# Kim-Dongjun/Soft-Truncation

Measured on AMD Instinct MI355X. Metric: training images/sec (DDPM++ CIFAR-10 32x32), higher is better.
Workload: dtype f32; 1 GPU; DDPM++ (VP) CIFAR-10 32x32, configs/vp/CIFAR10/ddpmpp_nll_st.py (BASELINE configs[1]); per_gpu_batch=128, global_batch=128, parallelism=dp1

## Files before the change

soft-truncation_amd/csrc/conv.hip:

```cpp
#include "igemm.h"
#include "stk_fp16.h"
#include "stk_fp16_train.h"

namespace {

using igemm::Cfg;
using igemm::MnMajor;
using igemm::keep_if;
using igemm::strip_row;

typedef __attribute__((address_space(1))) float gfloat;

struct ConvP {
  const float* x1; const float* x2; int C1, C2;
  const float* w; int w_layout;
  const float* bias; const float* temb; int temb_stride; const float* res; float inv_div; int use_div;
  float* y;
  const float* dy; float* dx1; float* dx2; float beta1, beta2, alpha;
  float* part; long part_stride;
  int N, H, W, Cin, Cout, OH, OW, KH, KW, stride, pad, sshift;
  int HW, OHW, taps;
  int ohw_shift, ow_shift;
};


template <int B, int KC, int LD>
struct RowChunk {
  static constexpr int PERQ = KC / 4, PASSES = B / 64, PER = PASSES * PERQ;
  static_assert(KC % 4 == 0 && B % 64 == 0 && PER <= 32, "bad RowChunk tile");
  const float* rowp[PASSES];
  unsigned rowbits;
  unsigned okm;
  int q, tid, Ktot;
  __device__ __forceinline__ void init(const float* base, long ld, int row0, int R, int Ktot_, int tid_) {
    tid = tid_; q = tid & 3; Ktot = Ktot_; rowbits = 0; okm = 0;
#pragma unroll
    for (int ps = 0; ps < PASSES; ++ps) {
      const int row = row0 + (tid >> 2) + 64 * ps;
      const bool ok = row < R;
      rowbits |= (ok ? 1u : 0u) << ps;
      rowp[ps] = base + (ok ? (long)row * ld : 0);
    }
  }
  __device__ __forceinline__ void load(int k0, float (&r)[PER]) {
    const int kb = k0 + q * PERQ;
    const bool kin = kb + PERQ <= Ktot;
    const int ko = kin ? kb : 0;
    okm = 0;
#pragma unroll
    for (int ps = 0; ps < PASSES; ++ps) {
      const float* s = rowp[ps] + ko;
#pragma unroll
      for (int j = 0; j < PERQ; ++j) r[ps * PERQ + j] = s[j];
      okm |= ((kin && ((rowbits >> ps) & 1u)) ? ((1u << PERQ) - 1u) : 0u) << (ps * PERQ);
    }
  }
  __device__ __forceinline__ void store(const float (&r)[PER], float* t) {
    if (okm == (PER == 32 ? 0xffffffffu : (1u << PER) - 1u)) {
#pragma unroll
      for (int ps = 0; ps < PASSES; ++ps)
#pragma unroll
        for (int j = 0; j < PERQ; ++j) t[(q * PERQ + j) * LD + (tid >> 2) + 64 * ps] = r[ps * PERQ + j];
    } else {
#pragma unroll
      for (int ps = 0; ps < PASSES; ++ps)
#pragma unroll
        for (int j = 0; j < PERQ; ++j)
          t[(q * PERQ + j) * LD + (tid >> 2) + 64 * ps] = keep_if(r[ps * PERQ + j], okm, ps * PERQ + j);
    }
  }
};

template <int B, int KC, int LD>
struct MnStrided {
  using Mp = MnMajor<B, KC>;
  static constexpr int PER = Mp::PER;
  const float* pm; long sk; int kg, tid, Ktot; bool ok;
  unsigned okm;
  __device__ __forceinline__ void init(const float* base, long smn, long sk_, int o0, int lim, int Ktot_, int tid_) {
    tid = tid_; sk = sk_; Ktot = Ktot_; okm = 0;
    const int mn = o0 + Mp::mn(tid);
    ok = mn < lim;
    pm = base + (ok ? (long)mn * smn : 0);
    kg = Mp::kgroup(tid) * PER;
  }
  __device__ __forceinline__ void load(int k0, float (&r)[PER]) {
    okm = 0;
#pragma unroll
    for (int i = 0; i < PER; ++i) {
      const int k = k0 + kg + i;
      const bool v = ok && k < Ktot;
      r[i] = pm[v ? (long)k * sk : 0];
      okm |= (v ? 1u : 0u) << i;
    }
  }
  __device__ __forceinline__ void store(const float (&r)[PER], float* t) {
#pragma unroll
    for (int i = 0; i < PER; ++i) t[(kg + i) * LD + Mp::mn(tid)] = keep_if(r[i], okm, i);
  }
};

template <class C>
struct AFwdK {
  RowChunk<C::BM, C::KC, C::LDA> rc;
  __device__ void init(const ConvP& p, int m0, int tid, int) { rc.init(p.w, (long)p.Cin * p.taps, m0, p.Cout, p.Cin * p.taps, tid); }
  __device__ void load(const ConvP&, int k0, float (&r)[C::NA]) { rc.load(k0, r); }
  __device__ void store(const float (&r)[C::NA], float* t) { rc.store(r, t); }
};
template <class C>
struct AFwdGen {
  MnStrided<C::BM, C::KC, C::LDA> ms;
  __device__ void init(const ConvP& p, int m0, int tid, int) { ms.init(p.w, (long)p.Cin * p.taps, 1, m0, p.Cout, p.Cin * p.taps, tid); }
  __device__ void load(const ConvP&, int k0, float (&r)[C::NA]) { ms.load(k0, r); }
  __device__ void store(const float (&r)[C::NA], float* t) { ms.store(r, t); }
};
template <class C>
struct AFwdNin {
  MnStrided<C::BM, C::KC, C::LDA> ms;
  __device__ void init(const ConvP& p, int m0, int tid, int) { ms.init(p.w, 1, p.Cout, m0, p.Cout, p.Cin, tid); }
  __device__ void load(const ConvP&, int k0, float (&r)[C::NA]) { ms.load(k0, r); }
  __device__ void store(const float (&r)[C::NA], float* t) { ms.store(r, t); }
};
template <class C>
struct ADgradNin {
  RowChunk<C::BM, C::KC, C::LDA> rc;
  __device__ void init(const ConvP& p, int m0, int tid, int) { rc.init(p.w, p.Cout, m0, p.Cin, p.Cout, tid); }
  __device__ void load(const ConvP&, int k0, float (&r)[C::NA]) { rc.load(k0, r); }
  __device__ void store(const float (&r)[C::NA], float* t) { rc.store(r, t); }
};
template <class C>
struct ADgradNinGen {
  MnStrided<C::BM, C::KC, C::LDA> ms;
  __device__ void init(const ConvP& p, int m0, int tid, int) { ms.init(p.w, p.Cout, 1, m0, p.Cin, p.Cout, tid); }
  __device__ void load(const ConvP&, int k0, float (&r)[C::NA]) { ms.load(k0, r); }
  __device__ void store(const float (&r)[C::NA], float* t) { ms.store(r, t); }
};
template <class C>
struct ADgrad1 {
  MnStrided<C::BM, C::KC, C::LDA> ms;
  __device__ void init(const ConvP& p, int m0, int tid, int) { ms.init(p.w, 1, p.Cin, m0, p.Cin, p.Cout, tid); }
  __device__ void load(const ConvP&, int k0, float (&r)[C::NA]) { ms.load(k0, r); }
  __device__ void store(const float (&r)[C::NA], float* t) { ms.store(r, t); }
};
template <class C>
struct ADgrad9 {
  static_assert(C::KC == 36, "3x3 chunks are 4 channels x 9 taps");
  static constexpr int PASSES = C::BM / 64;
  int m0, tid; unsigned okp;
  __device__ void init(const ConvP&, int m0_, int tid_, int) { m0 = m0_; tid = tid_; okp = 0; }
  __device__ void load(const ConvP& p, int k0, float (&r)[C::NA]) {
    const int co = k0 / 9 + (tid & 3);
    okp = 0;
#pragma unroll
    for (int ps = 0; ps < PASSES; ++ps) {
      const int m = m0 + (tid >> 2) + 64 * ps;
      const bool ok = m < p.Cin && co < p.Cout;
      const float* s = p.w + (ok ? ((long)co * p.Cin + m) * 9 : 0);
#pragma unroll
      for (int j = 0; j < 9; ++j) r[ps * 9 + j] = s[j];
      okp |= (ok ? 1u : 0u) << ps;
    }
  }
  __device__ void store(const float (&r)[C::NA], float* t) {
#pragma unroll
    for (int ps = 0; ps < PASSES; ++ps)
#pragma unroll
      for (int j = 0; j < 9; ++j)
        t[((tid & 3) * 9 + j) * C::LDA + (tid >> 2) + 64 * ps] = keep_if(r[ps * 9 + j], okp, ps);
  }
};

template <class C, int TAPS, bool DUAL>
// ... 169 lines not shown
    for (int i = 0; i < C::NB; ++i) {
      if (DUAL) {
        const bool f = (first >> i) & 1u;
        const uintptr_t tensor = f ? (uintptr_t)p.x1 : (uintptr_t)p.x2;
        r[i] = ((const gfloat*)tensor)[(f ? b1 : b2) + roff[i]];
      } else {
        r[i] = p.x1[b1 + roff[i]];
      }
    }
  }
  __device__ void store(const float (&r)[C::NB], float* t) {
#pragma unroll
    for (int i = 0; i < C::NB; ++i) t[(tid & 31) * C::LDB + (tid >> 5) + 8 * i] = keep_if(r[i], okm, i);
  }
};

struct EpFwd {
  int b; int col_off;
  static constexpr int TEMB_IMGS = 9;
  float rb; float rt[5]; int m0 = 0, b0 = 0, nimg = 0, tb = 0;
  const float* sb = nullptr; const float* stm = nullptr;
  __device__ void preload(const ConvP& p, int m0_, int n0, int tn, int M, int Nn, int tid) {
    m0 = m0_; sb = nullptr; stm = nullptr;
    b0 = n0 / p.OHW;
    nimg = min(n0 + tn - 1, Nn - 1) / p.OHW - b0 + 1;
    rb = (p.bias && tid < 128 && m0 + tid < M) ? p.bias[m0 + tid] : 0.f;
#pragma unroll
    for (int k = 0; k < 5; ++k) {
      const int idx = tid + 256 * k, img = idx >> 7, r = idx & 127;
      rt[k] = (p.temb && nimg <= TEMB_IMGS && img < nimg && m0 + r < M) ? p.temb[(long)(b0 + img) * p.temb_stride + m0 + r] : 0.f;
    }
  }
  __device__ void stage(unsigned char* lds, int tid) {
    __syncthreads();
    float* s = reinterpret_cast<float*>(lds);
    if (tid < 128) s[tid] = rb;
#pragma unroll
    for (int k = 0; k < 5; ++k) {
      const int idx = tid + 256 * k;
      if (idx < TEMB_IMGS * 128) s[128 + idx] = rt[k];
    }
    __syncthreads();
    sb = s; stm = s + 128;
  }
  __device__ void init(const ConvP&, int, int) {}
  __device__ void finish(const ConvP&, unsigned char*, int) {}
  __device__ void col(const ConvP& p, int n) {
    b = n / p.OHW;
    col_off = b * p.Cout * p.OHW + (n - b * p.OHW);
    tb = (b - b0) * 128;
  }
  __device__ void strip(const ConvP& p, int mbase, int M, bool nok, int, const floatx16& acc) {
    if (sb && (!p.temb || nimg <= TEMB_IMGS)) {
      const int ml = mbase - m0;
      float rv[16]; int idx[16];
#pragma unroll
      for (int e = 0; e < 16; ++e) {
        const int m = mbase + strip_row(e);
        const bool ok = nok && m < M;
        idx[e] = ok ? col_off + m * p.OHW : -1;
        rv[e] = (p.res && ok) ? p.res[idx[e]] : 0.f;
      }
#pragma unroll
      for (int g = 0; g < 4; ++g) {
        const float4 bb = *reinterpret_cast<const float4*>(sb + ml + 8 * g);
        const float4 tt = *reinterpret_cast<const float4*>(stm + tb + ml + 8 * g);
        const float bv[4] = {bb.x, bb.y, bb.z, bb.w}, tv[4] = {tt.x, tt.y, tt.z, tt.w};
#pragma unroll
        for (int u = 0; u < 4; ++u) {
          float v = acc[4 * g + u];
          if (p.bias) v += bv[u];
          if (p.temb) v += tv[u];
          if (p.res) v += rv[4 * g + u];
          if (p.use_div) v *= p.inv_div;
          if (idx[4 * g + u] >= 0) p.y[idx[4 * g + u]] = v;
        }
      }
      return;
    }
#pragma unroll
    for (int g = 0; g < 4; ++g) {
      float bv[4], tv[4], rv[4];
      int idx[4]; bool ok[4];
#pragma unroll
      for (int u = 0; u < 4; ++u) {
        const int m = mbase + strip_row(4 * g + u);
        ok[u] = nok && m < M;
        idx[u] = ok[u] ? col_off + m * p.OHW : 0;
        const int ms = ok[u] ? m : 0;
        bv[u] = p.bias ? p.bias[ms] : 0.f;
        tv[u] = p.temb ? p.temb[ok[u] ? (long)b * p.temb_stride + m : 0] : 0.f;
        rv[u] = p.res ? p.res[idx[u]] : 0.f;
      }
#pragma unroll
      for (int u = 0; u < 4; ++u) {
        float v = acc[4 * g + u];
        if (p.bias) v += bv[u];
        if (p.temb) v += tv[u];
        if (p.res) v += rv[u];
        if (p.use_div) v *= p.inv_div;
        if (ok[u]) p.y[idx[u]] = v;
      }
    }
  }
};
struct EpDgrad {
  int b, hw;
  __device__ void preload(const ConvP&, int, int, int, int, int, int) {}
  __device__ void stage(unsigned char*, int) {}
  __device__ void init(const ConvP&, int, int) {}
  __device__ void col(const ConvP& p, int n) { b = n / p.HW; hw = n - b * p.HW; }
  __device__ void strip(const ConvP& p, int mbase, int M, bool nok, int, const floatx16& acc) {
    const bool acc1 = p.beta1 != 0.f, acc2 = p.beta2 != 0.f;
#pragma unroll
    for (int e0 = 0; e0 < 16; e0 += 4) {
      float* d[4]; float old[4];
#pragma unroll
      for (int u = 0; u < 4; ++u) {
        const int m = mbase + strip_row(e0 + u);
        float* q = nullptr;
        if (nok && m < M) {
          if (m < p.C1) { if (p.dx1) q = p.dx1 + ((long)b * p.C1 + m) * p.HW + hw; }
          else if (p.dx2) q = p.dx2 + ((long)b * p.C2 + (m - p.C1)) * p.HW + hw;
        }
        d[u] = q;
        old[u] = 0.f;
        if (acc1 || acc2) {
          const float beta = m < p.C1 ? p.beta1 : p.beta2;
          if (q && beta != 0.f) old[u] = beta * *q;
        }
      }
#pragma unroll
      for (int u = 0; u < 4; ++u)
        if (d[u]) *d[u] = old[u] + p.alpha * acc[e0 + u];
    }
  }
  __device__ void finish(const ConvP&, unsigned char*, int) {}
};
struct EpWgrad {
  float* slab; int tap;
  __device__ void init(const ConvP& p, int zb, int zs) { slab = p.part + (long)zs * p.part_stride; tap = zb; }
  __device__ void col(const ConvP&, int) {}
  __device__ void strip(const ConvP& p, int mbase, int M, bool nok, int n, const floatx16& acc) {
#pragma unroll
    for (int e = 0; e < 16; ++e) {
      const int m = mbase + strip_row(e);
      if (nok && m < M) {
        slab[((long)tap * p.Cout + m) * p.Cin + n] = acc[e];
      }
    }
  }
};

struct EpSlab {
  float* slab; int Nn;
  __device__ void preload(const ConvP&, int, int, int, int, int, int) {}
  __device__ void stage(unsigned char*, int) {}
  __device__ void init(const ConvP& p, int, int zs) { slab = p.part + (long)zs * p.part_stride; Nn = p.N * p.HW; }
  __device__ void finish(const ConvP&, unsigned char*, int) {}
  __device__ void col(const ConvP&, int) {}
  __device__ void strip(const ConvP&, int mbase, int M, bool nok, int n, const floatx16& acc) {
#pragma unroll
    for (int e = 0; e < 16; ++e) {
      const int m = mbase + strip_row(e);
      if (nok && m < M) slab[(long)m * Nn + n] = acc[e];
    }
  }
};
template <class EP> struct OneProduct : EP {};
template <class EP> struct is_x1 { static constexpr bool value = false; };
template <class EP> struct is_x1<OneProduct<EP>> { static constexpr bool value = true; };
template <int VEC>
__global__ __launch_bounds__(256) void slab_fwd_kernel(ConvP p, int splits, int M, int Nn) {
  const long total = (long)M * Nn / VEC, gstride = (long)gridDim.x * 256;
  for (long iv = (long)blockIdx.x * 256 + threadIdx.x; iv < total; iv += gstride) {
    const long i = iv * VEC;
    const int m = (int)(i / Nn), n = (int)(i - (long)m * Nn);
    float v[VEC];
#pragma unroll
    for (int u = 0; u < VEC; ++u) v[u] = 0.f;
    for (int z = 0; z < splits; ++z) {
      const float* q = p.part + (long)z * p.part_stride + i;
      if constexpr (VEC == 4) {
        const float4 t = *reinterpret_cast<const float4*>(q);
        v[0] += t.x; v[1] += t.y; v[2] += t.z; v[3] += t.w;
      } else {
        v[0] += q[0];
      }
    }
    const int b = n / p.OHW;
    const long idx = ((long)b * p.Cout + m) * p.OHW + (n - b * p.OHW);
    float r[VEC];
#pragma unroll
    for (int u = 0; u < VEC; ++u) r[u] = 0.f;
    if (p.res) {
      if constexpr (VEC == 4) { const float4 t = *reinterpret_cast<const float4*>(p.res + idx); r[0] = t.x; r[1] = t.y; r[2] = t.z; r[3] = t.w; }
      else r[0] = p.res[idx];
    }
#pragma unroll
    for (int u = 0; u < VEC; ++u) {
      float w = v[u];
      if (p.bias) w += p.bias[m];
      if (p.temb) w += p.temb[(long)b * p.temb_stride + m];
      if (p.res) w += r[u];
      if (p.use_div) w *= p.inv_div;
      v[u] = w;
    }
    if constexpr (VEC == 4) *reinterpret_cast<float4*>(p.y + idx) = make_float4(v[0], v[1], v[2], v[3]);
    else p.y[idx] = v[0];
  }
}
template <int VEC>
__global__ __launch_bounds__(256) void slab_dgrad_kernel(ConvP p, int splits, int M, int Nn) {
  const long total = (long)M * Nn / VEC, gstride = (long)gridDim.x * 256;
  for (long iv = (long)blockIdx.x * 256 + threadIdx.x; iv < total; iv += gstride) {
    const long i = iv * VEC;
    const int m = (int)(i / Nn), n = (int)(i - (long)m * Nn);
    float v[VEC];
#pragma unroll
    for (int u = 0; u < VEC; ++u) v[u] = 0.f;
    for (int z = 0; z < splits; ++z) {
      const float* q = p.part + (long)z * p.part_stride + i;
      if constexpr (VEC == 4) {
        const float4 t = *reinterpret_cast<const float4*>(q);
        v[0] += t.x; v[1] += t.y; v[2] += t.z; v[3] += t.w;
      } else {
        v[0] += q[0];
      }
    }
    const int b = n / p.HW, hw = n - b * p.HW;
    float* d; float beta;
    if (m < p.C1) { d = p.dx1 ? p.dx1 + ((long)b * p.C1 + m) * p.HW + hw : nullptr; beta = p.beta1; }
    else { d = p.dx2 ? p.dx2 + ((long)b * p.C2 + (m - p.C1)) * p.HW + hw : nullptr; beta = p.beta2; }
    if (!d) continue;
    if constexpr (VEC == 4) {
      float4 o = make_float4(0.f, 0.f, 0.f, 0.f);
      if (beta != 0.f) { const float4 t = *reinterpret_cast<const float4*>(d); o = make_float4(beta * t.x, beta * t.y, beta * t.z, beta * t.w); }
      *reinterpret_cast<float4*>(d) = make_float4(o.x + p.alpha * v[0], o.y + p.alpha * v[1], o.z + p.alpha * v[2], o.w + p.alpha * v[3]);
    } else {
      *d = (beta != 0.f ? beta * *d : 0.f) + p.alpha * v[0];
    }
  }
}
inline void launch_slab_sum(const ConvP& p, int splits, int M, long Ng, int dgrad, hipStream_t s) {
  const bool al = stk_aligned16(p.part) && p.part_stride % 4 == 0 &&
                  (dgrad ? (p.HW % 4 == 0 && (!p.dx1 || stk_aligned16(p.dx1)) && (!p.dx2 || stk_aligned16(p.dx2)))
                         : (p.OHW % 4 == 0 && stk_aligned16(p.y) && (!p.res || stk_aligned16(p.res))));
  if (al && Ng % 4 == 0) {
    const dim3 rgrid((unsigned)stk_ew_grid((long)M * Ng / 4));
    if (dgrad) hipLaunchKernelGGL(slab_dgrad_kernel<4>, rgrid, dim3(256), 0, s, p, splits, M, (int)Ng);
    else hipLaunchKernelGGL(slab_fwd_kernel<4>, rgrid, dim3(256), 0, s, p, splits, M, (int)Ng);
  } else {
    const dim3 rgrid((unsigned)stk_ew_grid((long)M * Ng));
    if (dgrad) hipLaunchKernelGGL(slab_dgrad_kernel<1>, rgrid, dim3(256), 0, s, p, splits, M, (int)Ng);
    else hipLaunchKernelGGL(slab_fwd_kernel<1>, rgrid, dim3(256), 0, s, p, splits, M, (int)Ng);
  }
}

#include "conv_thin.h"
#include "conv_x2.h"
#include "conv_pl.h"
#include "conv_x2d.h"
#include "conv_x2w.h"

__device__ __forceinline__ long splitk_dst(long j, int layout, long CC, int Cout, int Cin, int taps) {
  if (layout == 0) {
    const int tap = (int)(j / CC);
    return (j - (long)tap * CC) * taps + tap;
  }
  const int co = (int)(j / Cin), ci = (int)(j - (long)co * Cin);
  return (long)ci * Cout + co;
}
__global__ __launch_bounds__(256) void splitk_reduce_kernel(const float* __restrict__ part, float* __restrict__ dw,
                                                            long n, int splits, long stride, float alpha, int layout,
                                                            int Cout, int Cin, int taps) {
  const long gstride = (long)gridDim.x * 256;
  const long CC = (long)Cout * Cin;
  const long n4 = ((n | stride) & 3) == 0 ? n / 4 : 0;
  for (long v = (long)blockIdx.x * 256 + threadIdx.x; v < n4; v += gstride) {
    const float4* src = reinterpret_cast<const float4*>(part) + v;
    float4 acc = {0.f, 0.f, 0.f, 0.f};
#pragma unroll 8
    for (int z = 0; z < splits; ++z) {
      const float4 t = src[(long)z * (stride / 4)];
      acc.x += t.x; acc.y += t.y; acc.z += t.z; acc.w += t.w;
    }
    const float a4[4] = {acc.x, acc.y, acc.z, acc.w};
#pragma unroll
    for (int e = 0; e < 4; ++e) dw[splitk_dst(4 * v + e, layout, CC, Cout, Cin, taps)] += alpha * a4[e];
  }
  for (long j = 4 * n4 + (long)blockIdx.x * 256 + threadIdx.x; j < n; j += gstride) {
    float sum = 0.f;
    for (int z = 0; z < splits; ++z) sum += part[(long)z * stride + j];
    dw[splitk_dst(j, layout, CC, Cout, Cin, taps)] += alpha * sum;
  }
}

__global__ __launch_bounds__(256) void splitk_reduce9_kernel(const float* __restrict__ part, float* __restrict__ dw, long CC,
                                                             int splits, long stride, float alpha) {
  __shared__ float s[256 * 9];
  const long q0 = (long)blockIdx.x * 256;
  const long q = q0 + threadIdx.x;
  const bool live = q < CC;
  float acc[9];
#pragma unroll
  for (int t = 0; t < 9; ++t) acc[t] = 0.f;
  const float* src = part + (live ? q : 0);
  int z = 0;
  for (; z + 4 <= splits; z += 4) {
    float v[4][9];
#pragma unroll
    for (int u = 0; u < 4; ++u)
#pragma unroll
      for (int t = 0; t < 9; ++t) v[u][t] = src[(long)(z + u) * stride + (long)t * CC];
#pragma unroll
    for (int u = 0; u < 4; ++u)
#pragma unroll
      for (int t = 0; t < 9; ++t) acc[t] += v[u][t];
  }
  for (; z < splits; ++z)
#pragma unroll
    for (int t = 0; t < 9; ++t) acc[t] += src[(long)z * stride + (long)t * CC];
#pragma unroll
  for (int t = 0; t < 9; ++t) s[threadIdx.x * 9 + t] = alpha * acc[t];
  __syncthreads();
  const long base = q0 * 9, end = CC * 9;
#pragma unroll
  for (int k = 0; k < 9; ++k) {
    const long i = base + k * 256 + threadIdx.x;
    if (i < end) dw[i] += s[k * 256 + threadIdx.x];
  }
}

template <int COLS>
__global__ __launch_bounds__(256) void wgrad9_kernel(ConvP p, int tiles_m, int tiles_n, int k_per_split) {
  constexpr int ROWS = 32 / COLS, TW = COLS + 2, TH = ROWS + 2, TSZ = TH * TW;
  constexpr int XS = TSZ | 1;
  constexpr int LDA = 129;
  constexpr int NX = (32 * TSZ + 255) / 256;
  constexpr int NA = 16;
  __shared__ float lds[32 * LDA + 32 * XS];
  float* As = lds;
  float* Xs = lds + 32 * LDA;

  const int tid = threadIdx.x, lane = tid & 63, wid = tid >> 6;
  const int fk = lane >> 5, fc = lane & 31;
  const int id = xcd_remap(blockIdx.x, gridDim.x);
  const int tn = id % tiles_n;
  const int rest = id / tiles_n;
  const int tm = rest % tiles_m, zs = rest / tiles_m;
  const int m0 = tm * 128, n0 = tn * 32;
  const int K = p.N * p.OHW;
  const int k_begin = zs * k_per_split;
  const int k_end = min(K, k_begin + k_per_split);

  const int mrow = m0 + (tid >> 5), cout_hi = p.Cout - 1;
  unsigned okrowsA = 0;
#pragma unroll
  for (int i = 0; i < NA; ++i) okrowsA |= (mrow + 8 * i < p.Cout ? 1u : 0u) << i;
  const int cin_hi = p.Cin - 1;
  floatx16 acc[9];
#pragma unroll
  for (int t = 0; t < 9; ++t)
#pragma unroll
    for (int e = 0; e < 16; ++e) acc[t][e] = 0.f;

  float ra[NA], rx[NX];
  unsigned okmA = 0, okmX = 0;
  auto load = [&](int k0) {
    const int k = k0 + (tid & 31);
    const bool kv = k < K;
    int b, ohw;
    split_pixel(p, kv ? k : 0, b, ohw);
    const int abase = b * p.Cout * p.OHW + ohw;
    okmA = kv ? okrowsA : 0u;
#pragma unroll
    for (int i = 0; i < NA; ++i) ra[i] = p.dy[abase + min(mrow + 8 * i, cout_hi) * p.OHW];
    int b0, ohw0, oy0, ox0;
    split_pixel(p, k0, b0, ohw0);
    split_row(p, ohw0, oy0, ox0);
    const int xbase = b0 * p.Cin * p.HW + (oy0 - 1) * p.W + (ox0 - 1);
    okmX = 0;
#pragma unroll
    for (int i = 0; i < NX; ++i) {
      const int e = tid + 256 * i;
      const int ci = e / TSZ, rem = e - ci * TSZ;
      const int lr = rem / TW, lc = rem - lr * TW;
      const int iy = oy0 - 1 + lr, ix = ox0 - 1 + lc;
      const bool ok = e < 32 * TSZ && n0 + ci < p.Cin && iy >= 0 && iy < p.H && ix >= 0 && ix < p.W;
      rx[i] = p.x1[ok ? xbase + min(n0 + ci, cin_hi) * p.HW + lr * p.W + lc : 0];
      okmX |= (ok ? 1u : 0u) << i;
    }
  };
  auto store = [&]() {
#pragma unroll
    for (int i = 0; i < NA; ++i) As[(tid & 31) * LDA + (tid >> 5) + 8 * i] = keep_if(ra[i], okmA, i);
#pragma unroll
    for (int i = 0; i < NX; ++i) {
      const int e = tid + 256 * i;
      const int ci = e / TSZ, rem = e - ci * TSZ;
      if (e < 32 * TSZ) Xs[ci * XS + rem] = keep_if(rx[i], okmX, i);
    }
  };

  if (k_begin < k_end) load(k_begin);
  const float* arow = As + fk * LDA + wid * 32 + fc;
  const float* xrow = Xs + fc * XS + fk;
  for (int k0 = k_begin; k0 < k_end; k0 += 32) {
    store();
// ... 109 lines not shown
    if (total > 0x7fffffffL) return STK_EUNSUPPORTED;
    hipLaunchKernelGGL((igemm::kernel<C, P, AL, BL, EP>), dim3((unsigned)total), dim3(256), 0, s, p, M, N, K, tm, tn,
                       k_per_split, batch);
  } else {
    dim3 grid((unsigned)(tm * tn), (unsigned)splits, (unsigned)batch);
    hipLaunchKernelGGL((igemm::kernel<C, P, AL, BL, EP>), grid, dim3(256), 0, s, p, M, N, K, tm, tn, k_per_split, 0);
  }
  STK_CHECK_LAUNCH();
  return STK_OK;
}

inline int fill_common(ConvP& p, int N, int H, int W, int C1, int C2, int Cout, int OH, int OW, int KH, int KW,
                       int stride, int pad) {
  if (N <= 0 || H <= 0 || W <= 0 || C1 <= 0 || C2 < 0 || Cout <= 0 || OH <= 0 || OW <= 0) return STK_EINVAL;
  if (!((KH == 3 && KW == 3) || (KH == 1 && KW == 1))) return STK_EUNSUPPORTED;
  if (stride != 1 && stride != 2) return STK_EUNSUPPORTED;
  const long lim = 0x7fffffffL;
  if ((long)N * (C1 > C2 ? C1 : C2) * H * W >= lim || (long)N * Cout * OH * OW >= lim) return STK_EUNSUPPORTED;
  p.N = N; p.H = H; p.W = W; p.C1 = C1; p.C2 = C2; p.Cin = C1 + C2; p.Cout = Cout; p.OH = OH; p.OW = OW;
  p.KH = KH; p.KW = KW; p.stride = stride; p.pad = pad; p.sshift = stride == 2 ? 1 : 0;
  p.HW = H * W; p.OHW = OH * OW; p.taps = KH * KW;
  p.ohw_shift = -1; p.ow_shift = -1;
  for (int sft = 0; sft < 31; ++sft) {
    if ((1 << sft) == p.OHW) p.ohw_shift = sft;
    if ((1 << sft) == p.OW) p.ow_shift = sft;
  }
  return STK_OK;
}

struct SplitPlan { int ok; int splits; int chunks_per_split; long slab; int t64; int gps; };
inline SplitPlan split_plan(const ConvP& p, int Kc, int S1, int S2, int M, long Ng) {
  SplitPlan r = {0, 1, 0, 0, 0, 0};
  const long big = (long)p.N * p.HW * 4 * (S1 > S2 ? S1 : S2);
  const bool geom = (p.taps == 9 && p.pad == 1) || (p.taps == 1 && p.pad == 0);
  if (!(big < 0x7fffffffL && geom && p.stride == 1 && p.OH == p.H && p.OW == p.W && Kc % 32 == 0 &&
        (S2 == 0 || S1 % 32 == 0) && M >= 96 && Ng <= 0x7fffffffL))
    return r;
  const long tiles = (long)stk_cdiv(M, 128) * stk_cdiv(Ng, 128);
  const int nch = p.taps * (Kc / 32);
  r.chunks_per_split = nch;
  if (tiles >= 192) { r.ok = 1; return r; }
  static const long target = [] { const char* e = getenv("STK_KSPLIT_WGS"); return e && atol(e) > 0 ? atol(e) : 512L; }();
  constexpr long minch = 12;
  long splits = target / tiles;
  const long mc = p.taps == 9 ? minch : (minch < 6 ? minch : 6);
  if (splits > nch / mc) splits = nch / mc;
  if ((tiles < 16 && p.taps != 9) || splits < 2) return r;
  r.chunks_per_split = (int)((nch + splits - 1) / splits);
  r.splits = (nch + r.chunks_per_split - 1) / r.chunks_per_split;
  r.slab = (long)M * Ng;
  r.ok = 1;
  return r;
}
inline SplitPlan fwd_split_plan(const ConvP& p) { return split_plan(p, p.Cin, p.C1, p.C2, p.Cout, (long)p.N * p.OHW); }
inline SplitPlan dgrad_split_plan(const ConvP& p) { return split_plan(p, p.Cout, p.Cout, 0, p.Cin, (long)p.N * p.HW); }
struct SplitWs { long xpart, part, bytes; };
inline long align256(long v) { return (v + 255) & ~255L; }
inline SplitWs split_ws(const SplitPlan& r, int M, int Kc, int taps) {
  SplitWs o;
  o.xpart = align256(x2::wp_bytes(M, Kc, taps));
  o.part = align256(o.xpart + 2L * x2::NPART * 4);
  o.bytes = r.ok ? 255 + o.part + (r.splits > 1 ? r.splits * r.slab * 4 : 0) : 0;
  return o;
}
inline void split_weight_strides(const ConvP& p, int dgrad, long& sm, long& sk) {
  if (p.w_layout == 0) { sm = dgrad ? p.taps : (long)p.Cin * p.taps; sk = dgrad ? (long)p.Cin * p.taps : p.taps; }
  else { sm = dgrad ? p.Cout : 1; sk = dgrad ? 1 : p.Cout; }
}
inline SplitPlan x1_plan(const SplitPlan& r, int nch1) {
  SplitPlan r1 = r;
  r1.chunks_per_split = (nch1 + r.splits - 1) / r.splits;
  r1.splits = (nch1 + r1.chunks_per_split - 1) / r1.chunks_per_split;
  return r1;
}

struct SplitGemm {
  ConvP p; x2::Src q; int M, Ng, tm, tn, nch, chunks_per_split; const float* xpart; int nx;
  bool dual, planes, halo; dim3 grid; hipStream_t s;
};
template <class E, int TAPS>
void split_gemm_taps(const SplitGemm& g) {
  constexpr bool X1 = is_x1<E>::value;
  if (!g.planes) {
    using A1 = std::conditional_t<X1, x2::ActLoader16<false, TAPS>, x2::ActLoader<false, TAPS>>;
    using A2 = std::conditional_t<X1, x2::ActLoader16<true, TAPS>, x2::ActLoader<true, TAPS>>;
    if (g.dual) hipLaunchKernelGGL((x2::gemm_kernel<A2, E>), g.grid, dim3(256), 0, g.s, g.p, g.q, g.M, g.Ng, g.tm, g.tn, g.nch,
                                   g.chunks_per_split, g.xpart, g.nx);
    else hipLaunchKernelGGL((x2::gemm_kernel<A1, E>), g.grid, dim3(256), 0, g.s, g.p, g.q, g.M, g.Ng, g.tm, g.tn, g.nch,
                            g.chunks_per_split, g.xpart, g.nx);
  } else if (g.halo) {
    if (g.p.W == 64)
      hipLaunchKernelGGL((x2d::gemm_halo_kernel<64, E, 1>), g.grid, dim3(256), 0, g.s, g.p, g.q, g.M, g.Ng, g.tm, g.tn, g.nch / 9, g.xpart, g.nx);
    else if (g.p.W == 32)
      hipLaunchKernelGGL((x2d::gemm_halo_kernel<32, E, 1>), g.grid, dim3(256), 0, g.s, g.p, g.q, g.M, g.Ng, g.tm, g.tn, g.nch / 9, g.xpart, g.nx);
    else
      hipLaunchKernelGGL((x2d::gemm_halo_kernel<16, E, 1>), g.grid, dim3(256), 0, g.s, g.p, g.q, g.M, g.Ng, g.tm, g.tn, g.nch / 9, g.xpart, g.nx);
  } else {
    hipLaunchKernelGGL((x2d::gemm_kernel<TAPS, 128, E>), g.grid, dim3(256), 0, g.s, g.p, g.q, g.M, g.Ng, g.tm, g.tn, g.nch,
                       g.chunks_per_split, g.xpart, g.nx);
  }
}
template <class E>
void split_gemm(const SplitGemm& g) {
  if (g.p.taps == 9) split_gemm_taps<E, 9>(g);
  else split_gemm_taps<E, 1>(g);
}

template <class EP>
int launch_split(ConvP p, const SplitPlan& r0, const float* s1, int S1, const float* s2, int S2, int M, long Ng, int dgrad,
                 void* ws, hipStream_t s, const void* wp_ready, float* amax, const void* planes, const float* planes_amax,
                 bool amax_valid, bool x1) {
  x2::Src q;
  q.s1 = s1; q.s2 = S2 > 0 ? s2 : s1; q.S1 = S1; q.S2 = S2; q.Kc = S1 + S2; q.Mpad = x2::pad128(M); q.taps = p.taps;
  q.pl = static_cast<const unsigned char*>(planes); q.pl_stride = planes ? pl::plane_bytes(p.N, S1, p.HW) : 0;
  const SplitWs lay = split_ws(r0, M, q.Kc, p.taps);
  unsigned char* base = reinterpret_cast<unsigned char*>(((uintptr_t)ws + 255) & ~(uintptr_t)255);
  float* xpart = reinterpret_cast<float*>(base + lay.xpart);
  p.part = reinterpret_cast<float*>(base + lay.part);
  p.part_stride = r0.slab;
  if (amax) xpart = amax + (dgrad ? 2 * x2::NPART : 0);
  if (planes) {
    xpart = const_cast<float*>(planes_amax);
  } else if (!(amax_valid && amax)) {
    hipLaunchKernelGGL(x2::amax_partial_kernel, dim3(x2::NPART), dim3(x2::AMAX_THREADS), 0, s, s1, (long)p.N * S1 * p.HW, xpart);
    if (S2 > 0)
      hipLaunchKernelGGL(x2::amax_partial_kernel, dim3(x2::NPART), dim3(x2::AMAX_THREADS), 0, s, s2, (long)p.N * S2 * p.HW,
                         xpart + x2::NPART);
    STK_CHECK_LAUNCH();
  }
  if (wp_ready) {
    q.wp = static_cast<const unsigned short*>(wp_ready);
  } else {
    x2::WprepDesc one = {};
    one.w = p.w; one.wp = base; one.M = M; one.Kc = q.Kc; one.Mpad = q.Mpad;
    one.taps = p.taps; one.flip = dgrad;
    split_weight_strides(p, dgrad, one.sm, one.sk);
    hipLaunchKernelGGL(x2::wamax_kernel, dim3(x2::WPART, 1), dim3(256), 0, s, nullptr, one);
    hipLaunchKernelGGL(x2::wprep_kernel, dim3((unsigned)stk_cdiv((long)q.Mpad * q.Kc, 256L)), dim3(256), 0, s, nullptr, one);
    STK_CHECK_LAUNCH();
    q.wp = reinterpret_cast<const unsigned short*>(base);
  }
  const int nch = planes && x1 ? p.taps * ((q.Kc / x2::KC + 1) / 2) : p.taps * (q.Kc / x2::KC);
  const SplitPlan r = planes && x1 ? x1_plan(r0, nch) : r0;
  SplitGemm g = {p, q, M, (int)Ng, q.Mpad / 128, stk_cdiv((int)Ng, 128), nch, r.chunks_per_split, xpart,
                 S2 > 0 ? 2 * x2::NPART : x2::NPART, S2 > 0, planes != nullptr, planes && x2d::halo_ok(p, p.taps, r0.splits),
                 dim3(), s};
  g.grid = dim3((unsigned)(g.tm * g.tn * r.splits));
  if (r0.splits == 1) {
    if (x1) split_gemm<OneProduct<EP>>(g);
    else split_gemm<EP>(g);
    STK_CHECK_LAUNCH();
    return STK_OK;
  }
  if (x1) split_gemm<OneProduct<EpSlab>>(g);
  else split_gemm<EpSlab>(g);
  STK_CHECK_LAUNCH();
  launch_slab_sum(p, r.splits, M, Ng, dgrad, s);
  STK_CHECK_LAUNCH();
  return STK_OK;
}

struct SplitWgradPlan { int ok; int splits; int chunks_per_split; long slab; int rows3; };
inline SplitWgradPlan split_wgrad_plan(int C1, int C2, int N, int Cout, int H, int W, int OH, int OW, int KH, int KW,
                                       int stride, int pad) {
  SplitWgradPlan q = {0, 0, 0, 0, 0};
  const int Cin = C1 + C2;
  const long K = (long)N * H * W;
  const int cmax = Cout > C1 ? (Cout > C2 ? Cout : C2) : (C1 > C2 ? C1 : C2);
  if (K * cmax * 4 >= 0x7fffffffL || (C2 > 0 && C1 % 32)) return q;
  const bool pow2 = (W & (W - 1)) == 0 && ((H * W) & (H * W - 1)) == 0;
  const bool geom = (KH == 3 && KW == 3 && pad == 1) || (KH == 1 && KW == 1 && pad == 0);
  if (!geom || stride != 1 || OH != H || OW != W || !pow2 || W < 4 || H * W < 16 || Cin < 64 || Cout < 64 ||
      K > 0x7fffffffL || K % 32)
    return q;
  const int taps = KH * KW;
  q.rows3 = (taps == 9 && W >= 8 && (C2 == 0 || C1 % 16 == 0)) ? 1 : 0;
  const long tiles = q.rows3 ? 3L * stk_cdiv(Cout, 128) * stk_cdiv(Cin, 64)
                             : (long)taps * stk_cdiv(Cout, 128) * stk_cdiv(Cin, 128);
  if (taps == 1 && tiles < 2) return q;
  const long chunks = K / 32;
  constexpr long w1_wgs = 256;
  long splits = (taps == 1 && tiles < 6 ? w1_wgs : 512) / tiles;
  if (splits > chunks / 8) splits = chunks / 8;
  if (splits < 1) splits = 1;
  q.chunks_per_split = (int)((chunks + splits - 1) / splits);
  q.splits = (int)((chunks + q.chunks_per_split - 1) / q.chunks_per_split);
  q.slab = (long)Cout * Cin * taps;
  q.ok = 1;
  return q;
}
template <int FORM>
void launch_x2w(const x2w::Args& a, int W, dim3 grid, hipStream_t s) {
  const dim3 block(256 * (FORM & 15));
  if (W >= 32) hipLaunchKernelGGL((x2w::wgrad_kernel<32, FORM>), grid, block, 0, s, a);
  else if (W == 16) hipLaunchKernelGGL((x2w::wgrad_kernel<16, FORM>), grid, block, 0, s, a);
  else if (W == 8) hipLaunchKernelGGL((x2w::wgrad_kernel<8, FORM>), grid, block, 0, s, a);
  else hipLaunchKernelGGL((x2w::wgrad_kernel<4, FORM>), grid, block, 0, s, a);
}
struct WgemmArgs {
  ConvP p; int tm, tn, nch, chunks_per_split; const float* dyp; const float* xp; int nx; dim3 grid; hipStream_t s;
};
template <bool X1, class BL>
void launch_wgemm_rows(const WgemmArgs& g) {
  using AL = std::conditional_t<X1, x2::RowsU16<false, false>, x2::RowsU<false, false>>;
  using E = std::conditional_t<X1, OneProduct<EpWgrad>, EpWgrad>;
  hipLaunchKernelGGL((x2::wgemm_kernel<AL, BL, E, !X1>), g.grid, dim3(256), 0, g.s, g.p, g.p.Cout, g.p.Cin, g.tm, g.tn, g.nch,
                     g.chunks_per_split, g.p.taps, g.dyp, g.xp, g.nx);
}
template <bool X1, bool DUAL>
void launch_wgemm_src(const WgemmArgs& g) {
  if (g.p.taps == 1)
    launch_wgemm_rows<X1, std::conditional_t<X1, x2::RowsU16<true, DUAL>, x2::RowsU<true, DUAL>>>(g);
  else if (g.p.W >= 16)
    launch_wgemm_rows<X1, std::conditional_t<X1, x2::RowsB16<DUAL, 16>, x2::RowsB<DUAL, 16>>>(g);
  else if (g.p.W == 8)
    launch_wgemm_rows<X1, std::conditional_t<X1, x2::RowsB16<DUAL, 8>, x2::RowsB<DUAL, 8>>>(g);
  else
    launch_wgemm_rows<X1, std::conditional_t<X1, x2::RowsB16<DUAL, 4>, x2::RowsB<DUAL, 4>>>(g);
}
template <bool X1>
void launch_wgemm(const WgemmArgs& g) {
  if (g.p.C2 > 0) launch_wgemm_src<X1, true>(g);
  else launch_wgemm_src<X1, false>(g);
}

struct WgradPlan { int big; int splits; int k_per_split; long slab; int mode9; };
inline int wgrad9_cols(int OH, int OW, int KH, int KW) {
  if (KH != 3 || KW != 3 || ((long)OH * OW) % 32 != 0) return 0;
  if (OW % 32 == 0) return 32;
  if (OW == 16 || OW == 8) return OW;
  return 0;
}
inline WgradPlan wgrad_plan(int Cin, int N, int Cout, int OH, int OW, int KH, int KW, bool allow9 = true) {
  WgradPlan q;
  q.mode9 = allow9 ? wgrad9_cols(OH, OW, KH, KW) : 0;
  if (q.mode9) {
    const long K = (long)N * OH * OW;
    const long tiles = (long)stk_cdiv(Cout, 128) * stk_cdiv(Cin, 32);
    const long chunks = K / 32;
    long splits = 256 / tiles;
    if (splits > chunks / 16) splits = chunks / 16;
    if (splits < 1) splits = 1;
    const long cps = (chunks + splits - 1) / splits;
    q.big = 1;
    q.k_per_split = (int)(cps * 32);
    q.splits = (int)((K + q.k_per_split - 1) / q.k_per_split);
    q.slab = (long)Cout * Cin * 9;
    return q;
  }
  const int taps = KH * KW;
  const long K = (long)N * OH * OW;
  const long tiles128 = (long)stk_cdiv(Cout, 128) * stk_cdiv(Cin, 128) * taps;
  q.big = (Cout >= 96 && Cin >= 96 && tiles128 >= 9) ? 1 : 0;
  const int T = q.big ? 128 : 64;
  const long tiles = (long)stk_cdiv(Cout, T) * stk_cdiv(Cin, T) * taps;
  const long chunks = (K + 31) / 32;
  long splits = (512 + tiles - 1) / tiles;
  if (splits > chunks / 16) splits = chunks / 16;
  if (splits < 1) splits = 1;
  const long cps = (chunks + splits - 1) / splits;
  q.k_per_split = (int)(cps * 32);
  q.splits = (int)((K + q.k_per_split - 1) / q.k_per_split);
  q.slab = (long)Cout * Cin * taps;
  return q;
}

}

extern "C" {

static int fwd_impl(const float* x1, int C1, const float* x2, int C2, const float* w, int w_layout,
                    const float* bias, const float* temb, int temb_stride, const float* res, float out_div,
                    float* y, int N, int H, int W, int Cout, int OH, int OW, int KH, int KW, int stride, int pad,
                    const void* wp, float* amax, void* ws, long ws_bytes, void* stream, bool x_rec_valid, bool f16x1) {
  if (!x1 || !w || !y || (C2 > 0 && !x2) || out_div == 0.f || (w_layout != 0 && w_layout != 1) ||
      (w_layout == 1 && (KH != 1 || KW != 1)))
    return STK_EINVAL;
  ConvP p = {};
  int rc = fill_common(p, N, H, W, C1, C2, Cout, OH, OW, KH, KW, stride, pad);
  if (rc) return rc;
  p.x1 = x1; p.x2 = C2 > 0 ? x2 : x1; p.w = w; p.w_layout = w_layout; p.bias = bias; p.temb = temb;
  p.temb_stride = temb_stride; p.res = res; p.inv_div = 1.f / out_div; p.use_div = out_div != 1.f; p.y = y;
  const int K = p.Cin * p.taps;
  const long Ng = (long)N * p.OHW;
  const bool big = use_big_tile(Cout, Ng, 1);
  hipStream_t s = (hipStream_t)stream;
  if (thin::geometry_ok(p) && Ng <= 0x7fffffffL) {
    const unsigned nblk = (unsigned)stk_cdiv(Ng, 256L);
    if (C2 == 0 && p.Cin <= 4) {
      thin::Args a = {x1, w, (long)p.Cin * p.taps, (long)p.taps, 0, p.Cin, Cout, p.taps, 0};
      const dim3 grid(nblk, (unsigned)stk_cdiv(Cout, thin::OB));
      if (p.taps == 9) hipLaunchKernelGGL((thin::thin_in_kernel<9>), grid, dim3(256), 0, s, p, a);
      else hipLaunchKernelGGL((thin::thin_in_kernel<1>), grid, dim3(256), 0, s, p, a);
      STK_CHECK_LAUNCH();
      return STK_OK;
    }
    if (Cout <= 4) {
      const unsigned nblk64 = (unsigned)stk_cdiv(Ng, 64L);
      if (p.taps == 9) hipLaunchKernelGGL((thin::thin_out_kernel<9>), dim3(nblk64), dim3(256), 0, s, p, Cout);
      else hipLaunchKernelGGL((thin::thin_out_kernel<1>), dim3(nblk64), dim3(256), 0, s, p, Cout);
      STK_CHECK_LAUNCH();
      return STK_OK;
    }
  }
  const SplitPlan xr = fwd_split_plan(p);
  if (ws && xr.ok && ws_bytes >= split_ws(xr, Cout, p.Cin, p.taps).bytes)
    return launch_split<EpFwd>(p, xr, x1, C1, x2, C2, Cout, Ng, 0, ws, s, wp, amax, nullptr, nullptr, x_rec_valid, f16x1);
  if (wp) return STK_EINVAL;
  if (p.taps == 9) {
// ... 557 lines not shown
```

soft-truncation_amd/csrc/conv_x2d.h:

```cpp
#pragma once

namespace x2d {

using x2::KC;
typedef __attribute__((address_space(3))) void lds_void;

template <int TN>
struct Geo {
  static constexpr int A_PLANE = 128 * 64, A_BYTES = 2 * A_PLANE;
  static constexpr int B_PLANE = TN * 64, B_BYTES = 2 * B_PLANE;
  static constexpr int LDS = A_BYTES + B_BYTES;
  static constexpr int NJ = TN / 64;
  static constexpr int BBLK = TN / 64;
};

__device__ __forceinline__ void dma16(__amdgpu_buffer_rsrc_t rs, unsigned char* dst, unsigned voff, unsigned soff) {
  __builtin_amdgcn_raw_ptr_buffer_load_lds(rs, (lds_void*)dst, 16, (int)voff, (int)soff, 0, 0);
}

template <int TAPS, int TN, class EP, int NBUF = 1, int ABL = 0>
__global__ __launch_bounds__(256, 2) void gemm_kernel(ConvP p, x2::Src q, int M, int Nn, int tiles_m, int tiles_n,
                                                      int nchunks_total, int chunks_per_split,
                                                      const float* __restrict__ xpart, int nxpart) {
  using G = Geo<TN>;
  constexpr bool X1 = is_x1<EP>::value;
  __shared__ __attribute__((aligned(1024))) unsigned char lds[G::LDS * NBUF];
  unsigned char* const As = lds;
  unsigned char* const Bs = lds + G::A_BYTES;
  const int tid = threadIdx.x;
  const int lane = tid & 63, wid = __builtin_amdgcn_readfirstlane(tid >> 6);
  __shared__ float red_amax[4];
  x2::LateAmax xmax;
  xmax.load(xpart, nxpart, tid);
  const float sw = x2::weight_scale(q.wp);
  const int ntiles = tiles_m * tiles_n;
  const int id = xcd_remap(blockIdx.x, gridDim.x);
  const int tile = id % ntiles, zs = id / ntiles;
  const int tm = tile % tiles_m, tn = tile / tiles_m;
  const int m0 = tm * 128, n0 = tn * TN;
  const int c_begin = zs * chunks_per_split;
  const int c_last = min(nchunks_total, c_begin + chunks_per_split) - 1;

  const unsigned seg_src = (unsigned)((lane & 3) ^ ((lane >> 4) & 3)) * 16u;
  const unsigned a_plane2 = (unsigned)q.taps * q.Mpad * q.Kc * 2u;
  const unsigned a_chunk2 = (unsigned)q.Mpad * KC * 2u;
  const __amdgpu_buffer_rsrc_t a_rs = x2::make_rsrc(reinterpret_cast<const unsigned char*>(q.wp) + x2::HEADER, 2L * a_plane2);
  const unsigned a_voff = (unsigned)(m0 + 32 * wid + (lane >> 2)) * 64u + seg_src;
  const __amdgpu_buffer_rsrc_t b_rs = x2::make_rsrc(q.pl, 2L * q.pl_stride);
  const unsigned b_ps = (unsigned)q.pl_stride;
  const int Cb = q.Kc >> 5;
  unsigned b_base[G::BBLK], b_mask[G::BBLK];
  {
#pragma unroll
    for (int jb = 0; jb < G::BBLK; ++jb) {
      const int n = n0 + (TN / 4) * wid + 16 * jb + (lane >> 2);
      b_mask[jb] = 0; b_base[jb] = 0;
      if (n < Nn) {
        const int b = n / p.HW, hw = n - b * p.HW;
        const int y = hw / p.W, x = hw - y * p.W;
        if (TAPS == 1) b_mask[jb] = 1u;
#pragma unroll
        for (int t = 0; t < (TAPS == 9 ? 9 : 0); ++t) {
          const int iy = y + t / 3 - 1, ix = x + t % 3 - 1;
          if (iy >= 0 && iy < p.H && ix >= 0 && ix < p.W) b_mask[jb] |= 1u << t;
        }
        b_base[jb] = ((unsigned)(b * Cb) * p.HW + hw) * 64u + seg_src;
      }
    }
  }
  auto stage = [&](int c, int buf = 0) {
    const int cc = TAPS == 9 ? c / 9 : c, tap = c - cc * TAPS;
    const unsigned a_soff = (unsigned)c * a_chunk2;
    unsigned char* const As = lds + buf * G::LDS;
    unsigned char* const Bs = As + G::A_BYTES;
    if (X1) {
#pragma unroll
      for (int s = 0; s < 2; ++s) {
        const unsigned dead = (2 * cc + s >= Cb) ? 0x80000000u : 0u;
#pragma unroll
        for (int h = 0; h < 2; ++h)
          dma16(a_rs, As + s * G::A_PLANE + (32 * wid + 16 * h) * 64, (a_voff + h * 1024u) | dead,
                (unsigned)((2 * cc + s) * TAPS + tap) * a_chunk2);
      }
    } else if (!(ABL & 2) || c == c_begin) {
#pragma unroll
    for (int s = 0; s < 2; ++s)
#pragma unroll
      for (int h = 0; h < 2; ++h)
        dma16(a_rs, As + s * G::A_PLANE + (32 * wid + 16 * h) * 64, a_voff + h * 1024u, a_soff + s * a_plane2);
    }
    const int shift = TAPS == 9 ? ((tap / 3 - 1) * p.W + (tap % 3 - 1)) * 64 : 0;
    const unsigned b_soff = (unsigned)cc * (unsigned)p.HW * 64u;
    if ((ABL & 1) && tap != 0) return;
#pragma unroll
    for (int jb = 0; jb < G::BBLK; ++jb) {
      const unsigned dead = (((b_mask[jb] >> tap) & 1u) ^ 1u) << 31;
      const unsigned vo = (b_base[jb] + (unsigned)shift) | dead;
#pragma unroll
      for (int s = 0; s < 2; ++s) {
        if (X1)
          dma16(b_rs, Bs + s * G::B_PLANE + ((TN / 4) * wid + 16 * jb) * 64, vo | (2 * cc + s >= Cb ? 0x80000000u : 0u),
                (unsigned)(2 * cc + s) * (unsigned)p.HW * 64u);
        else
          dma16(b_rs, Bs + s * G::B_PLANE + ((TN / 4) * wid + 16 * jb) * 64, vo, b_soff + s * b_ps);
      }
    }
  };

  EP ep;
  ep.preload(p, m0, n0, TN, M, Nn, tid);

  floatx16 acc[2][G::NJ];
#pragma unroll
  for (int i = 0; i < 2; ++i)
#pragma unroll
    for (int j = 0; j < G::NJ; ++j)
#pragma unroll
      for (int e = 0; e < 16; ++e) acc[i][j][e] = 0.f;

  const int wm0 = (wid & 1) * 64, wn0 = (wid >> 1) * (TN / 2);
  const int fk = lane >> 5, fc = lane & 31;
  const int fsw = (fc >> 2) & 3;
  const unsigned char* a_rd = As + (wm0 + fc) * 64;
  const unsigned char* b_rd = Bs + (wn0 + fc) * 64;
  const int ko0 = ((0 + fk) ^ fsw) * 16, ko1 = ((2 + fk) ^ fsw) * 16;

#define STK_D_FRAGS_AT(KO, OFF)                                                                           \
  _Pragma("unroll") for (int s = 0; s < 2; ++s) {                                                          \
    _Pragma("unroll") for (int i = 0; i < 2; ++i)                                                           \
      a[i][s] = *reinterpret_cast<const halfx8*>(a_rd + (OFF) + s * G::A_PLANE + i * 32 * 64 + (KO));      \
    _Pragma("unroll") for (int j = 0; j < G::NJ; ++j)                                                       \
      b[j][s] = *reinterpret_cast<const halfx8*>(b_rd + (OFF) + s * G::B_PLANE + j * 32 * 64 + (KO));      \
  }
#define STK_D_FRAGS(KO) STK_D_FRAGS_AT(KO, 0)
  constexpr int SA[3] = {1, 0, 0}, SB[3] = {0, 1, 0};
  constexpr int NPR = X1 ? 2 : 3;
#define STK_D_MFMAS                                                                                        \
  _Pragma("unroll") for (int pr = 0; pr < NPR; ++pr) _Pragma("unroll") for (int i = 0; i < 2; ++i)           \
    _Pragma("unroll") for (int j = 0; j < G::NJ; ++j) {                                                     \
      acc[i][j] = __builtin_amdgcn_mfma_f32_32x32x16_f16(a[i][X1 ? pr : SA[pr]], b[j][X1 ? pr : SB[pr]], acc[i][j], 0, 0, 0); \
    }

  halfx8 a[2][2], b[G::NJ][2];
  stage(c_begin);
  if constexpr (NBUF == 2) {
    int cur = 0;
    for (int c = c_begin; c <= c_last; ++c) {
      asm volatile("s_waitcnt vmcnt(0)" ::: "memory");
      __syncthreads();
      if (c < c_last) stage(c + 1, cur ^ 1);
      const int off = cur * G::LDS;
      STK_D_FRAGS_AT(ko0, off)
      STK_D_MFMAS
      STK_D_FRAGS_AT(ko1, off)
      STK_D_MFMAS
      cur ^= 1;
    }
  } else {
    for (int c = c_begin; c <= c_last; ++c) {
      asm volatile("s_waitcnt vmcnt(0)" ::: "memory");
      __syncthreads();
      if (!(ABL & 4) || c == c_begin) { STK_D_FRAGS(ko0) }
      STK_D_MFMAS
      if (!(ABL & 4) || c == c_begin) { STK_D_FRAGS(ko1) }
      __syncthreads();
      if (c < c_last) stage(c + 1);
      STK_D_MFMAS
    }
  }
#undef STK_D_MFMAS
#undef STK_D_FRAGS
#undef STK_D_FRAGS_AT

  const float unscale = 1.f / (sw * x2::pow2_scale_of(xmax.reduce(red_amax, tid)));
  ep.stage(lds, tid);
  ep.init(p, 0, zs);
#pragma unroll
  for (int j = 0; j < G::NJ; ++j) {
    const int n = n0 + wn0 + j * 32 + fc;
    const bool nok = n < Nn;
    ep.col(p, nok ? n : 0);
#pragma unroll
    for (int i = 0; i < 2; ++i) {
#pragma unroll
      for (int e = 0; e < 16; ++e) acc[i][j][e] *= unscale;
      ep.strip(p, m0 + wm0 + i * 32 + 4 * fk, M, nok, nok ? n : 0, acc[i][j]);
    }
  }
  ep.finish(p, lds, tid);
}
// ... 173 lines not shown
```

Measured before the change: 3371 images/s.

## Fuse split-K slab reduction into GEMM epilogue via per-tile ticket counters

Split-K GEMM blocks increment a per-output-tile atomic ticket after writing their partial slab. The last-arriving block then sums all splits and applies the forward (bias/temb/residual/divide) or dgrad (beta/alpha) epilogue itself, so the separate slab-sum kernel launch is skipped. Ticket counter sets are leased per scratch buffer from a device-global array. This removes one kernel launch and a full-grid pass per split-K conv, at the cost of release/acquire fences, a serialized tail reduction in one block per tile, and optional env knobs for tile-major ordering and atomic stores.

Result: slower. 3254 images/s (-3.5%).

```diff
diff --git a/soft-truncation_amd/csrc/conv.hip b/soft-truncation_amd/csrc/conv.hip
--- a/soft-truncation_amd/csrc/conv.hip
+++ b/soft-truncation_amd/csrc/conv.hip
@@ -1,4 +1,7 @@
+#include <mutex>
+
 #include "igemm.h"
+#include "ticket_lease.h"
 #include "stk_fp16.h"
 #include "stk_fp16_train.h"
 
@@ -18,6 +21,7 @@
   float* y;
   const float* dy; float* dx1; float* dx2; float beta1, beta2, alpha;
   float* part; long part_stride;
+  unsigned* ticket; int nsplit, slab_dgrad, slab_wt;
   int N, H, W, Cin, Cout, OH, OW, KH, KW, stride, pad, sshift;
   int HW, OHW, taps;
   int ohw_shift, ow_shift;
@@ -493,18 +497,127 @@
   }
 };
 
+typedef __attribute__((address_space(1))) unsigned gu32;
 struct EpSlab {
-  float* slab; int Nn;
-  __device__ void preload(const ConvP&, int, int, int, int, int, int) {}
+  float* slab; int Nn, m0, n0, M;
+  __device__ void preload(const ConvP&, int m0_, int n0_, int, int M_, int, int) { m0 = m0_; n0 = n0_; M = M_; }
   __device__ void stage(unsigned char*, int) {}
   __device__ void init(const ConvP& p, int, int zs) { slab = p.part + (long)zs * p.part_stride; Nn = p.N * p.HW; }
-  __device__ void finish(const ConvP&, unsigned char*, int) {}
   __device__ void col(const ConvP&, int) {}
-  __device__ void strip(const ConvP&, int mbase, int M, bool nok, int n, const floatx16& acc) {
+  __device__ void strip(const ConvP& p, int mbase, int M, bool nok, int n, const floatx16& acc) {
+    if (p.slab_wt & 1) {
+#pragma unroll
+      for (int e = 0; e < 16; ++e) {
+        const int m = mbase + strip_row(e);
+        if (nok && m < M) __hip_atomic_store(&slab[(long)m * Nn + n], acc[e], __ATOMIC_RELAXED, __HIP_MEMORY_SCOPE_AGENT);
+      }
+      return;
+    }
 #pragma unroll
     for (int e = 0; e < 16; ++e) {
       const int m = mbase + strip_row(e);
       if (nok && m < M) slab[(long)m * Nn + n] = acc[e];
+    }
+  }
+  __device__ void finish(const ConvP& p, unsigned char* lds, int tid) {
+    if (!p.ticket) return;
+    asm volatile("s_waitcnt vmcnt(0)" ::: "memory");
+    __syncthreads();
+    typedef __attribute__((address_space(3))) volatile unsigned lds_u32;
+    lds_u32* const last = (lds_u32*)lds;
+    if (tid == 0) {
+      if (!(p.slab_wt & 1)) {
+        __builtin_amdgcn_fence(__ATOMIC_RELEASE, "agent");
+        asm volatile("s_waitcnt vmcnt(0)" ::: "memory");
+      }
+      gu32* const t = (gu32*)(uintptr_t)p.ticket + ((m0 >> 7) + (n0 >> 7) * ((M + 127) >> 7));
+      const unsigned drew = __hip_atomic_fetch_add(t, 1u, __ATOMIC_RELAXED, __HIP_MEMORY_SCOPE_AGENT);
+      const unsigned is_last = drew == (unsigned)(p.nsplit - 1) ? 1u : 0u;
+      if (is_last) {
+        __hip_atomic_store(t, 0u, __ATOMIC_RELAXED, __HIP_MEMORY_SCOPE_AGENT);
+        __builtin_amdgcn_fence(__ATOMIC_ACQUIRE, "agent");
+        asm volatile("s_waitcnt vmcnt(0)" ::: "memory");
+      }
+      *last = is_last;
+    }
+    __syncthreads();
+    if (*last == 0u) return;
+    if (p.slab_dgrad) sum_tile<1>(p, tid);
+    else sum_tile<0>(p, tid);
+  }
+  template <int DG>
+  __device__ void sum_tile(const ConvP& p, int tid) const {
+    constexpr int RB = 8;
+    const int n = n0 + 4 * (tid & 31);
+    if (n >= Nn) return;
+    const int pix = DG ? p.HW : p.OHW;
+    const int b = n / pix, hw = n - b * pix;
+#pragma unroll 1
+    for (int k0 = 0; k0 < 16; k0 += RB) {
+      const int r0 = m0 + (tid >> 5) + 8 * k0;
+      float4 v[RB];
+#pragma unroll
+      for (int k = 0; k < RB; ++k) v[k] = make_float4(0.f, 0.f, 0.f, 0.f);
+#pragma unroll 1
+      for (int z = 0; z < p.nsplit; ++z) {
+        const float* const qz = p.part + (long)z * p.part_stride + n;
+        float4 t[RB];
+#pragma unroll
+        for (int k = 0; k < RB; ++k) {
+          const int m = r0 + 8 * k;
+          t[k] = *reinterpret_cast<const float4*>(qz + (long)(m < M ? m : m0) * Nn);
+        }
+#pragma unroll
+        for (int k = 0; k < RB; ++k) { v[k].x += t[k].x; v[k].y += t[k].y; v[k].z += t[k].z; v[k].w += t[k].w; }
+      }
+      if constexpr (DG == 0) {
+        float4 r[RB]; float bv[RB], tv[RB];
+#pragma unroll
+        for (int k = 0; k < RB; ++k) {
+          const int m = r0 + 8 * k, mv = m < M ? m : m0;
+          r[k] = make_float4(0.f, 0.f, 0.f, 0.f); bv[k] = 0.f; tv[k] = 0.f;
+          if (p.res) r[k] = *reinterpret_cast<const float4*>(p.res + ((long)b * p.Cout + mv) * p.OHW + hw);
+          if (p.bias) bv[k] = p.bias[mv];
+          if (p.temb) tv[k] = p.temb[(long)b * p.temb_stride + mv];
+        }
+#pragma unroll
+        for (int k = 0; k < RB; ++k) {
+          const int m = r0 + 8 * k;
+          float w[4] = {v[k].x, v[k].y, v[k].z, v[k].w};
+          const float rr[4] = {r[k].x, r[k].y, r[k].z, r[k].w};
+#pragma unroll
+          for (int u = 0; u < 4; ++u) {
+            if (p.bias) w[u] += bv[k];
+            if (p.temb) w[u] += tv[k];
+            if (p.res) w[u] += rr[u];
+            if (p.use_div) w[u] *= p.inv_div;
+          }
+          if (m < M) *reinterpret_cast<float4*>(p.y + ((long)b * p.Cout + m) * p.OHW + hw) = make_float4(w[0], w[1], w[2], w[3]);
+        }
+      } else {
+        float* d[RB]; float4 o[RB];
+        const bool olds = p.beta1 != 0.f || p.beta2 != 0.f;
+#pragma unroll
+        for (int k = 0; k < RB; ++k) {
+          const int m = r0 + 8 * k;
+          float beta = 0.f;
+          d[k] = nullptr;
+          if (m < M) {
+            if (m < p.C1) { d[k] = p.dx1 ? p.dx1 + ((long)b * p.C1 + m) * p.HW + hw : nullptr; beta = p.beta1; }
+            else { d[k] = p.dx2 ? p.dx2 + ((long)b * p.C2 + (m - p.C1)) * p.HW + hw : nullptr; beta = p.beta2; }
+          }
+          o[k] = make_float4(0.f, 0.f, 0.f, 0.f);
+          if (olds) {
+            const float4 t = *reinterpret_cast<const float4*>(d[k] ? d[k] : p.part);
+            if (d[k] && beta != 0.f) o[k] = make_float4(beta * t.x, beta * t.y, beta * t.z, beta * t.w);
+          }
+        }
+#pragma unroll
+        for (int k = 0; k < RB; ++k)
+          if (d[k])
+            *reinterpret_cast<float4*>(d[k]) = make_float4(o[k].x + p.alpha * v[k].x, o[k].y + p.alpha * v[k].y,
+                                                           o[k].z + p.alpha * v[k].z, o[k].w + p.alpha * v[k].w);
+      }
     }
   }
 };
@@ -583,11 +696,14 @@
     }
   }
 }
-inline void launch_slab_sum(const ConvP& p, int splits, int M, long Ng, int dgrad, hipStream_t s) {
+inline bool slab_sum_vec4(const ConvP& p, long Ng, int dgrad) {
   const bool al = stk_aligned16(p.part) && p.part_stride % 4 == 0 &&
                   (dgrad ? (p.HW % 4 == 0 && (!p.dx1 || stk_aligned16(p.dx1)) && (!p.dx2 || stk_aligned16(p.dx2)))
                          : (p.OHW % 4 == 0 && stk_aligned16(p.y) && (!p.res || stk_aligned16(p.res))));
-  if (al && Ng % 4 == 0) {
+  return al && Ng % 4 == 0;
+}
+inline void launch_slab_sum(const ConvP& p, int splits, int M, long Ng, int dgrad, hipStream_t s) {
+  if (slab_sum_vec4(p, Ng, dgrad)) {
     const dim3 rgrid((unsigned)stk_ew_grid((long)M * Ng / 4));
     if (dgrad) hipLaunchKernelGGL(slab_dgrad_kernel<4>, rgrid, dim3(256), 0, s, p, splits, M, (int)Ng);
     else hipLaunchKernelGGL(slab_fwd_kernel<4>, rgrid, dim3(256), 0, s, p, splits, M, (int)Ng);
@@ -596,6 +712,34 @@
     if (dgrad) hipLaunchKernelGGL(slab_dgrad_kernel<1>, rgrid, dim3(256), 0, s, p, splits, M, (int)Ng);
     else hipLaunchKernelGGL(slab_fwd_kernel<1>, rgrid, dim3(256), 0, s, p, splits, M, (int)Ng);
   }
+}
+
+
+__device__ unsigned g_ksplit_tickets[stk_lease::SETS * stk_lease::COUNTERS];
+inline int ksplit_fused_mode() {
+  const char* e = getenv("STK_KSPLIT_FUSED");
+  if (!e || !*e) return 1;
+  return e[0] == '0' ? 0 : e[0] == '2' ? 2 : 1;
+}
+inline unsigned* ksplit_tickets(const void* scratch) {
+  constexpr int MAXDEV = 64;
+  static stk_lease::Table table;
+  static std::mutex mu;
+  static unsigned* dev_base[MAXDEV] = {};
+  int dev = -1;
+  if (hipGetDevice(&dev) != hipSuccess || dev < 0 || dev >= MAXDEV) return nullptr;
+  unsigned* b;
+  {
+    std::lock_guard<std::mutex> lock(mu);
+    if (!dev_base[dev]) {
+      void* a = nullptr;
+      if (hipGetSymbolAddress(&a, HIP_SYMBOL(g_ksplit_tickets)) != hipSuccess) { (void)hipGetLastError(); return nullptr; }
+      dev_base[dev] = static_cast<unsigned*>(a);
+    }
+    b = dev_base[dev];
+  }
+  const int set = table.lease(reinterpret_cast<uintptr_t>(scratch));
+  return set < 0 ? nullptr : b + (long)set * stk_lease::COUNTERS;
 }
 
 #include "conv_thin.h"
@@ -1011,9 +1155,18 @@
     STK_CHECK_LAUNCH();
     return STK_OK;
   }
+  const int fused = g.planes && !g.halo ? ksplit_fused_mode() : 0;
+  if (fused) {
+    unsigned* const t = slab_sum_vec4(p, Ng, dgrad) && g.tm * g.tn <= stk_lease::COUNTERS ? ksplit_tickets(base) : nullptr;
+    if (!t && fused == 2) return STK_EUNSUPPORTED;
+    g.p.ticket = t; g.p.nsplit = r.splits; g.p.slab_dgrad = dgrad;
+    static const int wt = [] { const char* e = getenv("STK_KSPLIT_HANDOFF"); return e ? atoi(e) & 3 : 0; }();
+    g.p.slab_wt = t ? wt : 0;
+  }
   if (x1) split_gemm<OneProduct<EpSlab>>(g);
   else split_gemm<EpSlab>(g);
   STK_CHECK_LAUNCH();
+  if (g.p.ticket) return STK_OK;
   launch_slab_sum(p, r.splits, M, Ng, dgrad, s);
   STK_CHECK_LAUNCH();
   return STK_OK;
diff --git a/soft-truncation_amd/csrc/conv_x2d.h b/soft-truncation_amd/csrc/conv_x2d.h
--- a/soft-truncation_amd/csrc/conv_x2d.h
+++ b/soft-truncation_amd/csrc/conv_x2d.h
@@ -35,7 +35,8 @@
   const float sw = x2::weight_scale(q.wp);
   const int ntiles = tiles_m * tiles_n;
   const int id = xcd_remap(blockIdx.x, gridDim.x);
-  const int tile = id % ntiles, zs = id / ntiles;
+  const bool by_tile = p.ticket && (p.slab_wt & 2);
+  const int tile = by_tile ? id / p.nsplit : id % ntiles, zs = by_tile ? id % p.nsplit : id / ntiles;
   const int tm = tile % tiles_m, tn = tile / tiles_m;
   const int m0 = tm * 128, n0 = tn * TN;
   const int c_begin = zs * chunks_per_split;
diff --git a/soft-truncation_amd/csrc/ticket_lease.h b/soft-truncation_amd/csrc/ticket_lease.h
--- /dev/null
+++ b/soft-truncation_amd/csrc/ticket_lease.h
@@ -0,0 +1,31 @@
+#pragma once
+#include <cstdint>
+#include <mutex>
+
+namespace stk_lease {
+
+constexpr int SETS = 64;
+constexpr int COUNTERS = 256;
+
+class Table {
+ public:
+  int lease(uintptr_t addr) {
+    std::lock_guard<std::mutex> lock(mu_);
+    for (int i = 0; i < used_; ++i)
+      if (key_[i] == addr) return i;
+    if (used_ == SETS) return -1;
+    key_[used_] = addr;
+    return used_++;
+  }
+  int used() {
+    std::lock_guard<std::mutex> lock(mu_);
+    return used_;
+  }
+
+ private:
+  std::mutex mu_;
+  uintptr_t key_[SETS] = {};
+  int used_ = 0;
+};
+
+}
```
